# uw-math-ai/TheoremSearch

Hardware: AMD Instinct MI355X
Metric: queries/sec, brute-force top-10 over N x 768 theorem embeddings (higher is better)
Workload: dtype bf16; 1 GPU; 10000000x768 bf16 corpus, batch-256 queries, top-10 (BASELINE.json configs[2]); rows=10000000, dim=768, batch=256, k=10, searches_in_flight=1, parallelism=corpus row-sharded x1

## Files before the change

theoremsearch_amd/csrc/host.h:

```cpp
#pragma once
#include <hip/hip_runtime.h>

#include <algorithm>
#include <cmath>
#include <cctype>
#include <cstdarg>
#include <cstdio>
#include <cstdlib>
#include <cstring>
#include <atomic>
#include <memory>
#include <mutex>
#include <new>
#include <type_traits>
#include <vector>

#include "../../include/tsearch.h"
#include "common.h"
#include "scan_plan.h"
#include "anyd_plan.h"
#include "bias_plan.h"
#include "encoder_plan.h"
#include "meta_plan.h"
#include "dev_array.h"

using namespace ts;

inline thread_local char g_err[512] = "";

inline int fail(int code, const char* fmt, ...) {
    va_list ap;
    va_start(ap, fmt);
    vsnprintf(g_err, sizeof(g_err), fmt, ap);
    va_end(ap);
    return code;
}

#define HIP_TRY(expr)                                                                                   \
    do {                                                                                                \
        hipError_t e_ = (expr);                                                                         \
        if (e_ != hipSuccess)                                                                           \
            return fail(e_ == hipErrorOutOfMemory ? TS_ERR_NOMEM : TS_ERR_HIP, "%s failed: %s (%s:%d)", \
                        #expr, hipGetErrorString(e_), __FILE__, __LINE__);                              \
    } while (0)

#define DEV_TRY(expr) HIP_TRY((hipError_t)(expr))

#define TS_TRY(expr)            \
    do {                        \
        int rc_ = (expr);       \
        if (rc_ != TS_OK) return rc_; \
    } while (0)

template <auto Kernel, int Limit = 0, class... A>
inline int launch_lds(int dev, dim3 grid, dim3 block, int lds, hipStream_t st, const A&... args) {
    static std::atomic<int> raised[64];
    static std::mutex raise_mu;
    const int want = Limit ? Limit : lds;
    std::atomic<int>& have = raised[dev & 63];
    if (have.load(std::memory_order_acquire) < want) {
        std::lock_guard<std::mutex> lock(raise_mu);
        if (have.load(std::memory_order_relaxed) < want) {
            HIP_TRY(hipFuncSetAttribute((const void*)Kernel, hipFuncAttributeMaxDynamicSharedMemorySize, want));
            have.store(want, std::memory_order_release);
        }
    }
    Kernel<<<grid, block, lds, st>>>(args...);
    HIP_TRY(hipGetLastError());
    return TS_OK;
}

template <int V> using variant_c = std::integral_constant<int, V>;
template <int... Vs, class Go>
inline bool launch_variant(int variant, int* rc, Go&& go) {
    return ((variant == Vs && ((*rc = go(variant_c<Vs>{})), true)) || ...);
}

template <int... Vs, class Go>
inline int dispatch_value(int v, Go&& go) {
    int rc = TS_ERR_INVALID;
    if (!launch_variant<Vs...>(v, &rc, go)) return fail(rc, "internal: no kernel for the value %d", v);
    return rc;
}

enum Knob {
    K_MFMA_MIN_RANK, K_MFMA_VARIANT, K_MFMA_GROUPS, K_MFMA_GRID, K_MFMA_STAT, K_MFMA_STAT_CANDS, K_MFMA_TAIL_FIT,
    K_MFMA_NO_IDLE, K_MFMA_AHEAD, K_MFMA_TARGET_CANDS, K_MFMA_FIRST_ROWS, K_MFMA_TARGET_SPARSE, K_MFMA_RUN,
    K_MFMA_MIN_ROWS, K_MFMA_SHAPE, K_MFMA_F32, K_SCAN_GENERIC, K_SCAN_MAX_QUERIES, K_MFMA_BALANCE, K_PROBE_SPREAD, K_MFMA_SAMPLE,
    K_MFMA_PAIR, K_MFMA_PAIR_LAG, K_MFMA_SCREEN, K_MFMA_SCREEN_WIDE, K_MFMA_SCREEN_F32, K_MFMA_SCREEN_LATE, K_COUNT
};
inline const char* const kKnobNames[K_COUNT] = {
    "TS_MFMA_MIN_RANK", "TS_MFMA_VARIANT", "TS_MFMA_GROUPS", "TS_MFMA_GRID", "TS_MFMA_STAT", "TS_MFMA_STAT_CANDS",
    "TS_MFMA_TAIL_FIT", "TS_MFMA_NO_IDLE", "TS_MFMA_AHEAD", "TS_MFMA_TARGET_CANDS", "TS_MFMA_FIRST_ROWS",
    "TS_MFMA_TARGET_SPARSE", "TS_MFMA_RUN", "TS_MFMA_MIN_ROWS", "TS_MFMA_SHAPE", "TS_MFMA_F32", "TS_SCAN_GENERIC",
    "TS_SCAN_MAX_QUERIES", "TS_MFMA_BALANCE", "TS_PROBE_SPREAD", "TS_MFMA_SAMPLE", "TS_MFMA_PAIR", "TS_MFMA_PAIR_LAG",
    "TS_MFMA_SCREEN", "TS_MFMA_SCREEN_WIDE", "TS_MFMA_SCREEN_F32", "TS_MFMA_SCREEN_LATE"};
struct Knobs {
    int v[K_COUNT];
    bool set[K_COUNT];
    Knobs() {
        for (int i = 0; i < K_COUNT; ++i) {
            const char* e = getenv(kKnobNames[i]);
            set[i] = e && *e;
            v[i] = set[i] ? atoi(e) : 0;
        }
#ifndef TS_DIAG
        for (int i = 0; i < K_COUNT; ++i)
            if (diag_only((Knob)i)) { set[i] = false; v[i] = 0; }
#endif
    }
    static bool diag_only(Knob k) {
        return k == K_MFMA_VARIANT || k == K_MFMA_MIN_RANK || k == K_MFMA_GROUPS || k == K_MFMA_STAT_CANDS || k == K_MFMA_NO_IDLE ||
               k == K_MFMA_TARGET_CANDS || k == K_MFMA_TARGET_SPARSE || k == K_MFMA_MIN_ROWS || k == K_SCAN_GENERIC ||
               k == K_SCAN_MAX_QUERIES || k == K_PROBE_SPREAD;
    }
    int get(Knob k, int dflt) const { return set[k] ? v[k] : dflt; }
};

constexpr int kCandCap = 8192;
constexpr size_t kStageBytes = (size_t)256 << 20;

struct HipMem {
    static int alloc(void** p, size_t bytes) { return (int)hipMalloc(p, bytes ? bytes : 1); }
    static void free(void* p) { (void)hipFree(p); }
    static int zero(void* p, size_t bytes) { return (int)hipMemset(p, 0, bytes); }
};
template <class T> using DevArray = DevArrayOf<T, HipMem>;
using DevBuf = DevArray<void>;

struct IndexQueue {
    hipStream_t stream = nullptr;
    hipEvent_t order_ev = nullptr;
    bool ordered = false;
    std::vector<hipEvent_t> ev_pool;
    IndexQueue() = default;
    IndexQueue(const IndexQueue&) = delete;
    IndexQueue& operator=(const IndexQueue&) = delete;
    ~IndexQueue() {
        for (hipEvent_t e : ev_pool) hipEventDestroy(e);
        if (order_ev) hipEventDestroy(order_ev);
        if (stream) hipStreamDestroy(stream);
    }
};

struct ts_index : IndexQueue {
    int device = 0;
    int64_t n = 0, n_pad = 0, ld = 0, row_offset = 0;
    int d = 0, dtype = 0, metric = 0;
    int cu_count = 256;
    DevArray<void> rows;
    std::mutex mu;
    DevArray<void> stage;
    DevArray<void> qstore;      DevArray<float> qf32;
    DevArray<u64> cand;         DevArray<u32> count;         DevArray<float> thr;
    DevArray<u64> priv;         DevArray<u32> pcount;        int priv_writers = 0;
    DevArray<float> sample;
    bool rebalance_pending = false, rebalance_in_rerun = false; int rebalance_grid = 0;
    DevArray<int> fb_list;      DevArray<int> fb_count;      DevArray<u32> stat;
    DevArray<u64> partial;
    DevArray<u64> partial2;
    DevArray<float> res_scores; DevArray<int64_t> res_idx;   size_t res_cap = 0;
    DevArray<u32> mask_dev;
    DevArray<float> bias_dev;
    DevArray<u32> bias_hist;
    const float* active_bias = nullptr; float active_bias_w = 0.f;
    bool active_bias_matrix = false;
    DevArray<int64_t> id_map;
    bool borrowed = false;
    bool attached = false;
    ts_index* parent = nullptr;
    std::atomic<int> nviews{0};
    DevArray<void> rank_buf;
    DevArray<void> rank_many_buf;
    const u32* active_mask = nullptr;
    int64_t active_allowed = 0;
    Knobs knobs;
    hipStream_t last_stream = nullptr;
    DevArray<int64_t> part;     DevArray<unsigned> wg_ticks;
    int part_g = 0;             int64_t part_ntiles = -1;
// ... 53 lines not shown

inline hipEvent_t prof_begin(ts_index* ix, hipStream_t st, int64_t rows) {
    if (!ix->profiling) return nullptr;
    if (ix->ev_used + 2 > ix->ev_pool.size()) {
        if (ix->ev_pool.size() >= 16384) return nullptr;
        hipEvent_t a = nullptr, b = nullptr;
        if (hipEventCreate(&a) != hipSuccess) return nullptr;
        if (hipEventCreate(&b) != hipSuccess) { hipEventDestroy(a); return nullptr; }
        ix->ev_pool.push_back(a);
        ix->ev_pool.push_back(b);
    }
    hipEvent_t start = ix->ev_pool[ix->ev_used], stop = ix->ev_pool[ix->ev_used + 1];
    ix->ev_used += 2;
    ix->prof_rows = rows;
    hipEventRecord(start, st);
    return stop;
}
inline void prof_end(hipEvent_t stop, hipStream_t st) {
    if (stop) hipEventRecord(stop, st);
}

struct StreamScope {
    ts_index* ix = nullptr;
    hipStream_t st = nullptr;
    ~StreamScope() {
        if (!ix || !ix->order_ev) return;
        hipStreamCaptureStatus cap = hipStreamCaptureStatusNone;
        if (hipStreamIsCapturing(st, &cap) != hipSuccess) (void)hipGetLastError();
        if (cap != hipStreamCaptureStatusNone) return;
        if (hipEventRecord(ix->order_ev, st) == hipSuccess) {
            ix->last_stream = st;
            ix->ordered = true;
        } else {
            (void)hipGetLastError();
        }
    }
};
inline int enter_stream(ts_index* ix, void* stream, hipStream_t* out, StreamScope* scope) {
    hipStream_t st = stream ? (hipStream_t)stream : ix->stream;
    if (!ix->order_ev) HIP_TRY(hipEventCreateWithFlags(&ix->order_ev, hipEventDisableTiming));
    if (ix->ordered && ix->last_stream != st) HIP_TRY(hipStreamWaitEvent(st, ix->order_ev, 0));
    scope->ix = ix;
    scope->st = st;
    *out = st;
    return TS_OK;
}

inline int check_device(int device) {
    int c = 0;
    ts_device_count(&c);
    if (c <= 0) return fail(TS_ERR_NODEVICE, "no HIP device visible (libtsearch has no CPU path)");
    if (device < 0 || device >= c) return fail(TS_ERR_INVALID, "device %d out of range [0, %d)", device, c);
    return TS_OK;
}

static inline bool mfma_dim(int d) { return d == 384 || d == 512 || d == 768 || d == 1024; }
static inline bool two_level_search(const ts_index* ix) {
    return ix->knobs.get(K_MFMA_STAT, 1) != 0 && ix->knobs.get(K_MFMA_SAMPLE, 1) != 0;
}
static inline bool anyd_index(const ts_index* ix) {
    if (ix->dtype == TS_F32 && ix->knobs.get(K_MFMA_F32, 16) == 0) return false;
    return ix->ld == ix->d && anyd_served(ix->dtype, ix->d, two_level_search(ix));
}
static inline bool bias_index(const ts_index* ix) {
    if (ix->dtype == TS_F32 && ix->knobs.get(K_MFMA_F32, 16) == 0) return false;
    return ix->ld == ix->d && ix->n >= 1 && bias_served(ix->dtype, ix->d, two_level_search(ix));
}
static inline bool mfma_index(const ts_index* ix) {
    if (anyd_index(ix)) return true;
    if (ix->dtype == TS_BF16) return mfma_dim(ix->d);
    if (ix->knobs.get(K_MFMA_F32, 16) == 0) return false;
    return ix->d == 768 || ix->d == 1024 || ((ix->d == 384 || ix->d == 512) && two_level_search(ix));
}

static inline bool use_shape16(const ts_index* ix) {
    if (!mfma_dim(ix->d)) return false;
    const bool narrow = ix->d == 384 || ix->d == 512;
    const bool two_level = two_level_search(ix);
    if (ix->dtype == TS_F32) return ix->d != 768 || ix->knobs.get(K_MFMA_F32, 16) != 32;
    if (narrow && !two_level) return false;
    return ix->dtype == TS_BF16 && mfma_dim(ix->d) && ix->knobs.get(K_MFMA_SHAPE, 16) != 32;
}

namespace ts { struct MfmaArgs; }
int prep_dispatch(int src_dtype, int dst_dtype, bool normalize, const void* src, int64_t src_ld, void* dst, float* f32copy,
                  int64_t ld, int d, int64_t nrows, int64_t rows_total, hipStream_t st);
int scan_search(ts_index* ix, int nq, int k, float* out_scores, int64_t* out_idx, const int* qlist, const int* qcount,
                hipStream_t st, const float* qbuf = nullptr, const unsigned short* qb16 = nullptr);
struct QueryFeed {
    ts_index* ix = nullptr;
    const char* queries = nullptr;
    size_t row_bytes = 0;
    int q_dtype = 0;
    bool on_device = false, f32copy = false;
    hipStream_t st = nullptr;
    const void* at(int q0) const { return queries + (size_t)q0 * row_bytes; }
};
int query_feed_open(QueryFeed* f, ts_index* ix, const void* queries, int q_dtype, int q_on_device, int nq, bool f32copy, hipStream_t st);
int query_feed_block(const QueryFeed& f, int q0, int nb);
int mfma_block_queries(const ts_index* ix, int nq);
int bias_histogram(ts_index* ix, hipStream_t st);
int mfma_search(ts_index* ix, int nq, int k, float* out_scores, int64_t* out_idx, hipStream_t st, ts_search_stats* stats,
                const void* qmat, bool in_place);
int launch_pass_mfma16(int dev, int d, int nb, bool full_pass, int variant, int grid, hipStream_t st, const ts::MfmaArgs& a);
int launch_pass_mfma16_f32(int dev, int d, int nb, bool full_pass, int grid, hipStream_t st, const ts::MfmaArgs& a);
bool screen_usable(const ts_index* ix);
int screen_prepare(ts_index* ix, const void* qmat, int nq_launch, bool quantize_queries, hipStream_t st);
int screen_full_pass(ts_index* ix, int nb, int nq, int grid, int variant, bool ksplit, hipStream_t st, const ts::MfmaArgs& a);
int screen_tile_pass(ts_index* ix, int nb, int grid, int variant, hipStream_t st, const ts::MfmaArgs& a);
int screen_prepare_wide(ts_index* ix, const void* qmat, int nq_launch, bool quantize_queries, hipStream_t st);
int screen_full_pass_wide(ts_index* ix, int nb, int nq, int grid, int variant, bool ksplit, hipStream_t st, const ts::MfmaArgs& a);
int screen_tile_pass_wide(ts_index* ix, int nb, int grid, int variant, hipStream_t st, const ts::MfmaArgs& a);
int launch_screen8_late(int dev, int grid, hipStream_t st, const ts::MfmaArgs& a);
int screen_prepare_f32(ts_index* ix, const void* qmat, int nq_launch, hipStream_t st);
int screen_full_pass_f32(ts_index* ix, int nb, int nq, int grid, int variant, hipStream_t st, const ts::MfmaArgs& a);
int launch_pass_mfma_anyd(const ts_index* ix, int grid, hipStream_t st, const ts::MfmaArgs& a);
int launch_pass_mfma_anyd_biased(const ts_index* ix, int grid, hipStream_t st, const ts::MfmaArgs& a);
int launch_pass_mfma32(int dev, int d, int groups, bool full_pass, int variant, int grid, hipStream_t st, const ts::MfmaArgs& a);
int launch_pass_mfma32_f32(int dev, bool full_pass, int variant, int grid, hipStream_t st, const ts::MfmaArgs& a);
```

theoremsearch_amd/csrc/kernels_level.h:

```cpp
#pragma once
#include "kernels_select.h"

namespace ts {

struct LevelArgs {
    const u64* priv;
    const u32* pcount;
    int nwriters;
    int priv_cap;
    const u64* cand;
    u32* count;
    int cap;
    int kk;
    float* thr;
    int final_level;
    float z_tail;
    float tail_p;
    float tail_z;
    int min_fill;
    float* out_scores;
    int64_t* out_idx;
    int k_user;
    int64_t row_offset;
    const int64_t* id_map;
// ... 49 lines not shown
    TS_DPP_F64_STEP(TS_DPP_BCAST15, 0xa)
    TS_DPP_F64_STEP(TS_DPP_BCAST31, 0xc)
#undef TS_DPP_F64_STEP
    const u64 b = (u64)__double_as_longlong(v);
    const u32 lo = (u32)__builtin_amdgcn_readlane((int)(u32)b, 63), hi = (u32)__builtin_amdgcn_readlane((int)(u32)(b >> 32), 63);
    return __longlong_as_double((long long)(((u64)hi << 32) | lo));
}

constexpr int kFinalFast = 128;

__device__ __forceinline__ bool level_final_one_wave(const LevelArgs& a, int q) {
    if (!(a.final_level && a.nwriters == 0 && a.k_user <= kFinalFast)) return false;
    const u32 raw0 = a.count[q];
    if (!(raw0 <= (u32)kFinalFast && raw0 <= (u32)a.cap)) return false;
    if (threadIdx.x >= 64) return true;
    const int lane = threadIdx.x;
    u64 v[2];
#pragma unroll
    for (int r = 0; r < 2; ++r) v[r] = ((u32)(64 * r + lane) < raw0) ? a.cand[(int64_t)q * a.cap + 64 * r + lane] : 0ull;
    if (lane == 0) {
        a.count[q] = 0;
        a.stat_q[q] = raw0;
    }
    if ((int)raw0 < a.min_fill) {
        if (lane == 0) a.fb_list[atomicAdd(a.fb_count, 1)] = q;
        return true;
    }
    wave_sort_desc<u64, 2>(v, lane);
#pragma unroll
    for (int r = 0; r < 2; ++r) {
        const int i = 64 * r + lane;
        if (i < a.k_user) {
            const u64 key = v[r];
            a.out_scores[(int64_t)q * a.k_user + i] = key ? key_score(key) : -INFINITY;
            a.out_idx[(int64_t)q * a.k_user + i] = !key ? -1 : a.id_map ? a.id_map[key_row(key)] : (int64_t)key_row(key) + a.row_offset;
        }
    }
    return true;
}

template <int KR>
__global__ void __launch_bounds__(kLevelThreads) level_select_kernel(LevelArgs a) {
    extern __shared__ __attribute__((aligned(16))) unsigned char smem[];
    const SelectLds lds = SelectLds::carve(smem, kLevelSortMax);
    const int q = blockIdx.x;
    if (level_final_one_wave(a, q)) return;
    u32& fill = lds.ctr[kSelFill];
    u32& produced = lds.ctr[kSelProduced];
    u32& base_shared = lds.ctr[kSelSharedBase];
    if (threadIdx.x == 0) {
        fill = 0;
        produced = 0;
        lds.ctr[kSelShort] = 0;
    }
    for (int i = threadIdx.x; i < kLevelBins; i += blockDim.x) lds.hist[i] = 0;
    __syncthreads();
    for (int w = threadIdx.x; w < a.nwriters; w += blockDim.x) {
        const u32 made = a.pcount[(int64_t)q * a.nwriters + w];
        if (made == 0) continue;
        const u32 n = min(made, (u32)a.priv_cap);
        const u64* src = a.priv + ((int64_t)q * a.nwriters + w) * a.priv_cap;
        const u32 at = atomicAdd(&fill, n);
        atomicAdd(&produced, n);
        u64 v[32];
#pragma unroll
        for (int e = 0; e < 32; ++e) v[e] = ((u32)e < n) ? src[e] : 0ull;
#pragma unroll
        for (int e = 0; e < 32; ++e)
            if ((u32)e < n && at + e < (u32)kLevelSortMax) lds.keys[at + e] = v[e];
    }
    const u32 raw = a.count[q];
    const u32 ns = min(raw, (u32)a.cap);
    __syncthreads();
    if (threadIdx.x == 0) {
        base_shared = fill;
        fill += ns;
        produced += raw;
    }
    __syncthreads();
    for (u32 i = threadIdx.x; i < ns; i += blockDim.x)
        if (base_shared + i < (u32)kLevelSortMax) lds.keys[base_shared + i] = a.cand[(int64_t)q * a.cap + i];
    __syncthreads();
    const u32 total = fill;
    const bool lost = raw > (u32)a.cap || total > (u32)kLevelSortMax;
    const int cnt = (int)min(total, (u32)kLevelSortMax);
    const int kk = a.kk;
    constexpr int kTailM = 32;
    const bool tail_fit = !a.final_level && a.tail_p > 0.0f;
    const int kl = tail_fit ? max(kk, kTailM) : kk;

    double mean = 0.0, sd = 0.0;
    u64* best = lds_select_top<KR>(lds, cnt, kl, !a.final_level && a.z_tail > 0.0f && cnt >= 256, mean, sd);

    if (threadIdx.x == 0) a.count[q] = 0;
    if (!a.final_level) {
        const float thr = level_threshold(a, best, cnt, kk, tail_fit, mean, sd);
        if (threadIdx.x == 0) a.thr[q] = thr;
        return;
    }
    if (threadIdx.x == 0) a.stat_q[q] = produced;
    if (lost || (int)total < a.min_fill) {
        if (threadIdx.x == 0) a.fb_list[atomicAdd(a.fb_count, 1)] = q;
        return;
    }
    for (int i = threadIdx.x; i < a.k_user; i += blockDim.x) {
        const u64 key = best[i];
        a.out_scores[(int64_t)q * a.k_user + i] = key ? key_score(key) : -INFINITY;
        a.out_idx[(int64_t)q * a.k_user + i] = !key ? -1 : a.id_map ? a.id_map[key_row(key)] : (int64_t)key_row(key) + a.row_offset;
    }
}

constexpr int kSelCap = 1024;

constexpr int kSelThreads = 256;
template <int THREADS>
__global__ void __launch_bounds__(THREADS) sample_select_fast_kernel(LevelArgs a, const float* scores, int row_stride, float z_sel) {
    constexpr int NW = THREADS / 64;
    constexpr int J4 = kLevelSortMax / (4 * THREADS);
    __shared__ double red[2 * NW];
    __shared__ u32 wcount[2][NW];
    __shared__ __attribute__((aligned(16))) u32 surv[kSelCap];
    __shared__ __attribute__((aligned(16))) u64 best[kSelCap];
    __shared__ u32 nsurv;
    const int q = blockIdx.x;
    const int lane = threadIdx.x & 63, wave = threadIdx.x >> 6;
    if (threadIdx.x == 0) {
        a.count[q] = 0;
        nsurv = 0;
    }
    const float4* src = (const float4*)(scores + (int64_t)q * row_stride);
    const int n4 = row_stride >> 2;
    float v[4 * J4];
#pragma unroll
    for (int j = 0; j < J4; ++j) {
        const int i = j * THREADS + threadIdx.x;
        const float4 t = (i < n4) ? src[i] : make_float4(-INFINITY, -INFINITY, -INFINITY, -INFINITY);
        v[4 * j] = t.x; v[4 * j + 1] = t.y; v[4 * j + 2] = t.z; v[4 * j + 3] = t.w;
    }
    double s1 = 0.0, s2 = 0.0;
    u32 nl = 0;
    u32 o[4 * J4];
#pragma unroll
    for (int e = 0; e < 4 * J4; ++e) {
        const bool live = v[e] == v[e] && v[e] > -INFINITY;
        const double d = live ? (double)v[e] : 0.0;
        s1 += d;
        s2 += d * d;
        nl += (u32)__popcll(__ballot(live));
        o[e] = live ? ord_f32(v[e]) : 0u;
    }
    s1 = wave_total_f64(s1);
    s2 = wave_total_f64(s2);
    if (lane == 0) { red[2 * wave] = s1; red[2 * wave + 1] = s2; wcount[0][wave] = nl; }
    __syncthreads();
    double t1 = 0.0, t2 = 0.0;
    int cnt = 0;
#pragma unroll
    for (int w = 0; w < NW; ++w) { t1 += red[2 * w]; t2 += red[2 * w + 1]; cnt += (int)wcount[0][w]; }
    const double mean = cnt > 0 ? t1 / cnt : 0.0;
    const double sd = cnt > 0 ? sqrt(fmax(t2 / cnt - mean * mean, 0.0)) : 0.0;
    const int kk = a.kk;
    constexpr int kTailM = 32;
    const bool tail_fit = a.tail_p > 0.0f;
    const int kl = min(tail_fit ? max(kk, kTailM) : kk, kMaxK);

    int flip = 1;
    auto count_ge = [&](u32 cut) __attribute__((always_inline)) -> u32 {
        u32 c = 0;
#pragma unroll
        for (int e = 0; e < 4 * J4; ++e) c += (u32)__popcll(__ballot(o[e] >= cut));
        if (lane == 0) wcount[flip][wave] = c;
        __syncthreads();
        u32 tot = 0;
#pragma unroll
        for (int w = 0; w < NW; ++w) tot += wcount[flip][w];
        flip ^= 1;
        return tot;
    };
    const u32 want = (u32)min(kl, cnt);
    u32 cut = 1u, c = 0;
    bool found = want == 0;
    if (!found && sd > 0.0) {
        float z = z_sel;
        for (int t = 0; t < 3 && !found; ++t) {
            cut = max(ord_f32((float)(mean + (double)z * sd)), 1u);
            c = count_ge(cut);
            if (c < want) z -= 0.75f;
            else if (c > (u32)kSelCap) z += 0.75f;
            else found = true;
        }
    }
    if (!found) {
// ... 64 lines not shown
```

theoremsearch_amd/csrc/launch_screen8.hip:

```cpp
#include "launch_screen8_impl.h"

bool screen_usable(const ts_index* ix) {
    bool served = false;
    if (ix->dtype == TS_BF16) served = ix->d == 768 || (ix->d == 1024 && ix->knobs.get(K_MFMA_SCREEN_WIDE, 0) != 0);
    else if (ix->dtype == TS_F32)
        served = (ix->d == 768 || ix->d == 1024) && ix->knobs.get(K_MFMA_SCREEN_F32, 0) != 0 && ix->knobs.get(K_MFMA_F32, 16) != 32 &&
                 two_level_search(ix);
    return served && ix->ld == ix->d && use_shape16(ix) && !ix->borrowed && !ix->attached && ix->knobs.get(K_MFMA_SCREEN, 1) != 0;
}

int screen_prepare(ts_index* ix, const void* qmat, int nq_launch, bool quantize_queries, hipStream_t st) {
    if (ix->dtype == TS_F32) return screen_prepare_f32(ix, qmat, nq_launch, st);
    if (ix->d == 1024) return screen_prepare_wide(ix, qmat, nq_launch, quantize_queries, st);
    return screen_prepare_w<768>(ix, qmat, nq_launch, quantize_queries, st);
}

int screen_full_pass(ts_index* ix, int nb, int nq, int grid, int variant, bool ksplit, hipStream_t st, const MfmaArgs& a) {
    if (ix->dtype == TS_F32) return screen_full_pass_f32(ix, nb, nq, grid, variant, st, a);
    if (ix->d == 1024) return screen_full_pass_wide(ix, nb, nq, grid, variant, ksplit, st, a);
    return screen_full_pass_w<768>(ix, nb, nq, grid, variant, ksplit, st, a);
}

int screen_tile_pass(ts_index* ix, int nb, int grid, int variant, hipStream_t st, const MfmaArgs& a) {
    if (ix->d == 1024) return screen_tile_pass_wide(ix, nb, grid, variant, st, a);
    return screen_tile_pass_w<768>(ix, nb, grid, variant, st, a);
}
```

theoremsearch_amd/csrc/launch_screen8_impl.h:

```cpp
#pragma once
#include "host.h"
#include "kernels_screen8.h"

template <int W, int NB>
static int launch_screen8(int dev, int grid, int variant, hipStream_t st, const MfmaArgs& a) {
    constexpr int D = W / 2;
    constexpr int lds = Mfma16Dims<D>::kLds + kMfma16StageBytes;
#ifdef TS_DIAG
    constexpr bool kDiag = NB == 4;
#else
    constexpr bool kDiag = false;
#endif
    static_assert(lds <= 160 * 1024, "DMA ring + staged candidates must fit the CU's LDS");
    const bool masked = a.row_mask != nullptr;
    auto go = [&](auto v) { return launch_lds<mfma16_topk_kernel<D, NB, decltype(v)::value, false>>(dev, grid, kMfmaThreads, lds, st, a); };
    int rc;
    if constexpr (kDiag)
        if (launch_variant<kVariantScreenNoEpilogue, kVariantScreenStamps, kVariantScreenClockProbe, kVariantScreenDmaOnly, kVariantScreenTestOnly>(variant, &rc, go)) return rc;
    return masked ? go(variant_c<kVariantScreenMasked>{}) : go(variant_c<kVariantScreen>{});
}

template <int W, class QuantizeTiles, class QuantizeQueries>
static int screen_prepare_with(ts_index* ix, bool quantize_queries, QuantizeTiles&& quantize_tiles, QuantizeQueries&& quantize_query_rows) {
    const int64_t tiles = ix->n_pad / kTileRows;
    if (ix->scr_pad != ix->n_pad) {
        ix->scr_pad = 0;
        DEV_TRY(remake(ix->scr_rows, (size_t)ix->n_pad * W, ix->scr_tile, (size_t)tiles * 16));
        ix->scr_pad = ix->n_pad;
        ix->scr_lo = 0;
        ix->scr_hi = ix->n_pad;
    }
    if (ix->scr_lo < ix->scr_hi) {
        const int64_t t0 = ix->scr_lo / kTileRows;
        const int64_t t1 = std::min(tiles, (ix->scr_hi + kTileRows - 1) / kTileRows);
        for (int64_t t = t0; t < t1; t += 1 << 20) {
            quantize_tiles(t, (unsigned)std::min<int64_t>(1 << 20, t1 - t));
            HIP_TRY(hipGetLastError());
        }
        ix->scr_lo = ix->scr_hi = 0;
    }
    DEV_TRY(ix->scr_q.need((size_t)kMfmaQ * W));
    DEV_TRY(ix->scr_qmeta.need((size_t)kMfmaQ * 16));
    DEV_TRY(ix->scr_cand.need((size_t)kMfmaQ * kScreenCap * 8));
    DEV_TRY(ix->scr_count.need((size_t)kMfmaQ * 4));
    if (quantize_queries) {
        quantize_query_rows();
        HIP_TRY(hipGetLastError());
    }
    return TS_OK;
}

template <int W>
static int screen_prepare_w(ts_index* ix, const void* qmat, int nq_launch, bool quantize_queries, hipStream_t st) {
    return screen_prepare_with<W>(
        ix, quantize_queries,
        [&](int64_t tile0, unsigned nblk) {
            quantize_tiles_kernel<W><<<nblk, 256, 0, st>>>(ix->rows.as<const unsigned short>(), ix->scr_rows.as<signed char>(), ix->scr_tile.as<float4>(), tile0);
        },
        [&] {
            quantize_queries_kernel<W><<<kMfmaQ, 64, 0, st>>>((const unsigned short*)qmat, std::min(nq_launch, kMfmaQ), ix->scr_q.as<signed char>(),
                                                           ix->scr_qmeta.as<float4>(), ix->scr_count);
        });
}

template <int W>
static int screen_tile_pass_w(ts_index* ix, int nb, int grid, int variant, hipStream_t st, const MfmaArgs& a, bool late = false) {
    MfmaArgs s = a;
    s.corpus = ix->scr_rows.as<const unsigned short>();
    s.q = ix->scr_q.as<const unsigned short>();
    s.cand = ix->scr_cand;
    s.count = ix->scr_count;
    s.cap = kScreenCap;
    s.scr_tile = ix->scr_tile.as<const float4>();
    s.scr_q = ix->scr_qmeta.as<const float4>();
    if constexpr (W == 768)
        if (late && nb == 4 && variant == kVariantProduct && s.row_mask == nullptr) return launch_screen8_late(ix->device, grid, st, s);
    switch (nb) {
        case 1: return launch_screen8<W, 1>(ix->device, grid, variant, st, s);
        case 2: return launch_screen8<W, 2>(ix->device, grid, variant, st, s);
        case 3: return launch_screen8<W, 3>(ix->device, grid, variant, st, s);
        case 4: return launch_screen8<W, 4>(ix->device, grid, variant, st, s);
        default: return fail(TS_ERR_INTERNAL, "no int8 screen with %d query blocks per wave", nb);
    }
}

template <int W>
static int screen_full_pass_w(ts_index* ix, int nb, int nq, int grid, int variant, bool ksplit, hipStream_t st, const MfmaArgs& a) {
    TS_TRY(screen_tile_pass_w<W>(ix, nb, grid, variant, st, a, W == 768 && ix->dtype == TS_BF16 && ix->knobs.get(K_MFMA_SCREEN_LATE, 1) != 0));
    ScreenRescoreArgs r;
    r.rows = ix->rows.as<const unsigned short>();
    r.q = a.q;
    r.thr = a.thr;
    r.scand = ix->scr_cand;
    r.scount = ix->scr_count;
    r.cand = a.cand;
    r.count = a.count;
    r.cap = a.cap;
    if constexpr (W == 1024) {
        if (ksplit) screen_rescore_kernel<W, true><<<dim3((unsigned)nq, kRescoreY), 256, 0, st>>>(r);
        else screen_rescore_kernel<W, false><<<dim3((unsigned)nq, kRescoreY), 256, 0, st>>>(r);
    } else {
        if (ksplit) return fail(TS_ERR_INTERNAL, "the k-split rescore is a form of the d = 1024 pass, not of d = %d", W);
        screen_rescore_kernel<W, false><<<dim3((unsigned)nq, kRescoreY), 256, 0, st>>>(r);
    }
    HIP_TRY(hipGetLastError());
    return TS_OK;
}
```

theoremsearch_amd/csrc/search_mfma.hip:

```cpp
#include "host.h"
#include "kernels_mfma.h"
#include "kernels_mfma16.h"
#include "mfma16_variants.h"
#include "kernels_mfma_f32.h"
#include "kernels_sample.h"
#include "kernels_sample_biased.h"
#include "kernels_level.h"

struct Level { int64_t stride, ntiles; int run; };

static double normal_tail_z(double p) {
    if (p <= 0.0) return 8.0;
    if (p >= 0.5) return 0.0;
    const double q = std::sqrt(-2.0 * std::log(p));
    static const double c[] = {-7.784894002430293e-03, -3.223964580411365e-01, -2.400758277161838e+00,
                               -2.549732539343734e+00, 4.374664141464968e+00, 2.938163982698783e+00};
    static const double d[] = {7.784695709041462e-03, 3.224671290700398e-01, 2.445134137142996e+00, 3.754408661907416e+00};
    if (p < 0.02425)
        return -(((((c[0] * q + c[1]) * q + c[2]) * q + c[3]) * q + c[4]) * q + c[5]) /
               ((((d[0] * q + d[1]) * q + d[2]) * q + d[3]) * q + 1.0);
    static const double a[] = {-3.969683028665376e+01, 2.209460984245205e+02, -2.759285104469687e+02,
                               1.383577518672690e+02, -3.066479806614716e+01, 2.506628277459239e+00};
    static const double b[] = {-5.447609879822406e+01, 1.615858368580409e+02, -1.556989798598866e+02,
                               6.680131188771972e+01, -1.328068155288572e+01};
// ... 289 lines not shown
            ix->probe_units = (double)h[2];
            if (ix->knobs.get(K_PROBE_SPREAD, 0)) {
                std::vector<double> us;
                double xm[8] = {0}, xn[8] = {0};
                for (int w = 0; w < grid; ++w)
                    if (h[w * 4 + 1] > 0) {
                        us.push_back((double)h[w * 4 + 1] * 0.01);
                        xm[w & 7] += us.back();
                        xn[w & 7] += 1;
                    }
                std::sort(us.begin(), us.end());
                fprintf(stderr, "[tsearch probe] tile loop per workgroup: min %.1f us, median %.1f, max %.1f; mean by id %% 8:", us.front(),
                        us[us.size() / 2], us.back());
                for (int x = 0; x < 8; ++x) fprintf(stderr, " %.1f", xm[x] / std::max(1.0, xn[x]));
                fprintf(stderr, "\n");
            }
        }
    } else if (p.shape16 && (variant == kVariantStamps || (p.screen && variant == kVariantScreenStamps))) {
        std::vector<unsigned long long> h((size_t)grid * 16);
        HIP_TRY(hipStreamSynchronize(st));
        HIP_TRY(hipMemcpy(h.data(), dbg, h.size() * 8, hipMemcpyDeviceToHost));
        const double units = (double)(p.lv.back().ntiles * (variant == kVariantScreenStamps ? (ix->d == 1024 ? Mfma16Dims<512>::kUnits : Mfma16Dims<384>::kUnits) : MfmaDims<768>::kUnits)) / grid;
        for (int wv = 0; wv < 4; ++wv) {
            double tot = 0, vm = 0, bar = 0, dma = 0;
            for (int w = wv; w < grid * 4; w += 4) { tot += h[w * 4]; vm += h[w * 4 + 1]; bar += h[w * 4 + 2]; dma += h[w * 4 + 3]; }
            if (variant == kVariantScreenStamps)
                fprintf(stderr, "[tsearch stamps8] wave %d per tile: total %.0f cycles, vmcnt wait %.0f, barrier wait %.0f, tile tail %.0f (drain to end of epilogue; stamp cost ~40 each included)\n",
                        wv, tot / grid / units, vm / grid / units, bar / grid / units, dma / grid / units);
            else
                fprintf(stderr, "[tsearch stamps16] wave %d per unit: total %.0f cycles, vmcnt wait %.0f, barrier wait %.0f, DMA issue %.0f (6 pieces; stamp cost ~40 each included)\n",
                        wv, tot / grid / units, vm / grid / units, bar / grid / units, dma / grid / units);
        }
    } else if (!p.shape16) {
        std::vector<unsigned long long> h((size_t)grid * 16);
        HIP_TRY(hipStreamSynchronize(st));
        HIP_TRY(hipMemcpy(h.data(), dbg, h.size() * 8, hipMemcpyDeviceToHost));
        for (int wv = 0; wv < 4; ++wv) {
            double tot = 0, vm = 0, bar = 0, units = 0;
            for (int w = wv; w < grid * 4; w += 4) { tot += h[w * 4]; vm += h[w * 4 + 1]; bar += h[w * 4 + 2]; units += h[w * 4 + 3]; }
            fprintf(stderr, "[tsearch stamps] wave %d per unit: total %.0f cycles, vmcnt wait %.0f, barrier wait %.0f (units/wave %.0f)\n",
                    wv, tot / units, vm / units, bar / units, units / grid);
        }
    }
    return TS_OK;
}
#endif

static int mfma_level(ts_index* ix, const MfmaPlan& p, size_t i, int nq, int k, float* out_scores, int64_t* out_idx, const void* qmat,
                      hipStream_t st) {
    const Level& lv = p.lv[i];
    const bool full_pass = (i + 1 == p.lv.size());
    MfmaArgs a;
    a.corpus = ix->rows.as<const unsigned short>();
    a.n = ix->n;
    a.ntiles = lv.ntiles;
    a.tile_stride = lv.stride;
    a.run = lv.run;
    a.q = (const unsigned short*)qmat;
    a.thr = ix->thr;
    a.nq = ix->knobs.get(K_MFMA_NO_IDLE, 0) ? 256 : nq;
    a.row_mask = ix->active_mask;
    a.ahead = ix->knobs.get(K_MFMA_AHEAD, 0);
    a.priv = ix->priv;
    a.pcount = ix->pcount;
    a.cand = ix->cand;
    a.count = ix->count;
    a.cap = kCandCap;
    a.first_level = (i == 0) ? 1 : 0;
    a.nq_real = nq;
    a.fb_count = ix->fb_count;
    a.part = (p.balance && full_pass) ? ix->part : nullptr;
    a.wg_ticks = (p.balance && full_pass) ? ix->wg_ticks : nullptr;
    a.pair = (p.pair && full_pass) ? (p.ksplit_form ? 2 : 1) : 0;
    const bool paced = a.pair && p.pair_lag > 0;
    a.pair_pos = paced ? ix->pair_pos : nullptr;
    a.pair_lag = paced ? p.pair_lag : 0;
    a.dbg = nullptr;
    a.scr_tile = nullptr;
    a.scr_q = nullptr;
#ifdef TS_DIAG
    if (variant_gets_dbg(p.variant) && !p.anyd) a.dbg = ix->dbg;
#endif
    if (p.anyd && !full_pass) return fail(TS_ERR_INTERNAL, "the general-width matrix kernel has no sparse level");
    hipEvent_t stop = full_pass ? prof_begin(ix, st, ix->n) : nullptr;
    int rc;
    if (p.biased) rc = launch_pass_mfma_anyd_biased(ix, p.grid, st, a);
    else if (p.anyd) rc = launch_pass_mfma_anyd(ix, p.grid, st, a);
    else if (p.screen && full_pass) rc = screen_full_pass(ix, p.nb16, nq, p.grid, p.screen_diag ? p.variant : kVariantProduct, p.ksplit_form, st, a);
    else if (ix->dtype == TS_F32 && p.shape16) rc = launch_pass_mfma16_f32(ix->device, ix->d, p.nb16, full_pass, p.grid, st, a);
    else if (ix->dtype == TS_F32) rc = launch_pass_mfma32_f32(ix->device, full_pass, p.variant, p.grid, st, a);
    else if (p.shape16) rc = launch_pass_mfma16(ix->device, ix->d, p.nb16, full_pass, p.variant, p.grid, st, a);
    else rc = launch_pass_mfma32(ix->device, ix->d, p.groups, full_pass, p.variant, p.grid, st, a);
    prof_end(stop, st);
    TS_TRY(rc);
#ifdef TS_DIAG
    if (a.dbg && full_pass) TS_TRY(mfma_diag_readout(ix, p, a.dbg, st));
#endif
    LevelArgs l;
    memset(&l, 0, sizeof(l));
    l.priv = ix->priv;
    l.pcount = ix->pcount;
    l.nwriters = ((p.shape16 || p.anyd) && full_pass) ? 0 : p.nwriters;
    l.priv_cap = p.priv_cap;
    l.cand = ix->cand;
    l.count = ix->count;
    l.cap = kCandCap;
    l.kk = p.kk;
    l.thr = ix->thr;
    l.final_level = full_pass;
    l.z_tail = full_pass ? 0.0f : p.z_tail;
    l.tail_p = full_pass ? 0.0f : p.tail_p;
    l.tail_z = (float)normal_tail_z(std::min(0.25, 32.0 / p.sample_rows));
    l.min_fill = (int)std::min<int64_t>(k, p.pop);
    l.out_scores = out_scores;
    l.out_idx = out_idx;
    l.k_user = k;
    l.row_offset = ix->row_offset;
    l.id_map = ix->id_map;
    l.fb_list = ix->fb_list;
    l.fb_count = ix->fb_count;
    l.stat_q = ix->stat;
    l.nq = nq;
    if (p.kk <= 64) return launch_lds<level_select_kernel<1>>(ix->device, nq, kLevelThreads, kLevelLds, st, l);
    return launch_lds<level_select_kernel<4>>(ix->device, nq, kLevelThreads, kLevelLds, st, l);
}

int mfma_search(ts_index* ix, int nq, int k, float* out_scores, int64_t* out_idx, hipStream_t st, ts_search_stats* stats,
                       const void* qmat, bool in_place) {
    const MfmaPlan p = mfma_plan(ix, nq, k);
    TS_TRY(mfma_scratch(ix, p, st));
    if (p.screen) TS_TRY(screen_prepare(ix, qmat, p.nq_launch, !(p.dense0 && p.screen_rider), st));
    for (size_t i = 0; i < p.lv.size(); ++i) {
        if (i == 0 && p.dense0) TS_TRY(mfma_sample(ix, p, nq, qmat, st));
        else TS_TRY(mfma_level(ix, p, i, nq, k, out_scores, out_idx, qmat, st));
    }
    ix->rebalance_pending = p.balance;
    ix->rebalance_grid = p.wgs;
    ix->rebalance_in_rerun = !(p.dense_sample && p.lv.size() == 2);
    if (!in_place) TS_TRY(scan_search(ix, nq, k, out_scores, out_idx, ix->fb_list, ix->fb_count, st));
    else if (ix->dtype == TS_F32) TS_TRY(scan_search(ix, nq, k, out_scores, out_idx, ix->fb_list, ix->fb_count, st, (const float*)qmat));
    else TS_TRY(scan_search(ix, nq, k, out_scores, out_idx, ix->fb_list, ix->fb_count, st, nullptr, (const unsigned short*)qmat));
    if (stats) {
        stats->levels = (int)p.lv.size();
        stats->screened = p.screen ? 1 : 0;
    }
    return TS_OK;
}
```

Before: 156,200 queries/s.

## Fuse screened rescore and final top-k select into one finish kernel

For the bf16 d=768 screened search, the rescore of screened candidates and the final level select now run in a single kernel per query instead of two launches. Candidates are rescored with MFMA into LDS keys and selected in place, with a wave-sort fast path for small candidate counts, so the intermediate candidate list no longer round-trips through global memory and one launch is removed. The fused kernel uses 1024 threads and a large LDS footprint, which may lower occupancy compared with the separate rescore kernel.

```diff
diff --git a/theoremsearch_amd/csrc/host.h b/theoremsearch_amd/csrc/host.h
--- a/theoremsearch_amd/csrc/host.h
+++ b/theoremsearch_amd/csrc/host.h
@@ -87,14 +87,15 @@
     K_MFMA_MIN_RANK, K_MFMA_VARIANT, K_MFMA_GROUPS, K_MFMA_GRID, K_MFMA_STAT, K_MFMA_STAT_CANDS, K_MFMA_TAIL_FIT,
     K_MFMA_NO_IDLE, K_MFMA_AHEAD, K_MFMA_TARGET_CANDS, K_MFMA_FIRST_ROWS, K_MFMA_TARGET_SPARSE, K_MFMA_RUN,
     K_MFMA_MIN_ROWS, K_MFMA_SHAPE, K_MFMA_F32, K_SCAN_GENERIC, K_SCAN_MAX_QUERIES, K_MFMA_BALANCE, K_PROBE_SPREAD, K_MFMA_SAMPLE,
-    K_MFMA_PAIR, K_MFMA_PAIR_LAG, K_MFMA_SCREEN, K_MFMA_SCREEN_WIDE, K_MFMA_SCREEN_F32, K_MFMA_SCREEN_LATE, K_COUNT
+    K_MFMA_PAIR, K_MFMA_PAIR_LAG, K_MFMA_SCREEN, K_MFMA_SCREEN_WIDE, K_MFMA_SCREEN_F32, K_MFMA_SCREEN_LATE,
+    K_MFMA_FINISH, K_COUNT
 };
 inline const char* const kKnobNames[K_COUNT] = {
     "TS_MFMA_MIN_RANK", "TS_MFMA_VARIANT", "TS_MFMA_GROUPS", "TS_MFMA_GRID", "TS_MFMA_STAT", "TS_MFMA_STAT_CANDS",
     "TS_MFMA_TAIL_FIT", "TS_MFMA_NO_IDLE", "TS_MFMA_AHEAD", "TS_MFMA_TARGET_CANDS", "TS_MFMA_FIRST_ROWS",
     "TS_MFMA_TARGET_SPARSE", "TS_MFMA_RUN", "TS_MFMA_MIN_ROWS", "TS_MFMA_SHAPE", "TS_MFMA_F32", "TS_SCAN_GENERIC",
     "TS_SCAN_MAX_QUERIES", "TS_MFMA_BALANCE", "TS_PROBE_SPREAD", "TS_MFMA_SAMPLE", "TS_MFMA_PAIR", "TS_MFMA_PAIR_LAG",
-    "TS_MFMA_SCREEN", "TS_MFMA_SCREEN_WIDE", "TS_MFMA_SCREEN_F32", "TS_MFMA_SCREEN_LATE"};
+    "TS_MFMA_SCREEN", "TS_MFMA_SCREEN_WIDE", "TS_MFMA_SCREEN_F32", "TS_MFMA_SCREEN_LATE", "TS_MFMA_FINISH"};
 struct Knobs {
     int v[K_COUNT];
     bool set[K_COUNT];
@@ -314,7 +315,7 @@
     return ix->dtype == TS_BF16 && mfma_dim(ix->d) && ix->knobs.get(K_MFMA_SHAPE, 16) != 32;
 }
 
-namespace ts { struct MfmaArgs; }
+namespace ts { struct MfmaArgs; struct LevelArgs; struct ScreenRescoreArgs; }
 int prep_dispatch(int src_dtype, int dst_dtype, bool normalize, const void* src, int64_t src_ld, void* dst, float* f32copy,
                   int64_t ld, int d, int64_t nrows, int64_t rows_total, hipStream_t st);
 int scan_search(ts_index* ix, int nq, int k, float* out_scores, int64_t* out_idx, const int* qlist, const int* qcount,
@@ -338,7 +339,10 @@
 int launch_pass_mfma16_f32(int dev, int d, int nb, bool full_pass, int grid, hipStream_t st, const ts::MfmaArgs& a);
 bool screen_usable(const ts_index* ix);
 int screen_prepare(ts_index* ix, const void* qmat, int nq_launch, bool quantize_queries, hipStream_t st);
-int screen_full_pass(ts_index* ix, int nb, int nq, int grid, int variant, bool ksplit, hipStream_t st, const ts::MfmaArgs& a);
+int screen_full_pass(ts_index* ix, int nb, int nq, int grid, int variant, bool ksplit, hipStream_t st, const ts::MfmaArgs& a,
+                     const ts::LevelArgs* finish = nullptr);
+bool screen_finish_served(const ts_index* ix);
+int launch_screen_finish(int dev, int nq, hipStream_t st, const ts::ScreenRescoreArgs& r, const ts::LevelArgs& l);
 int screen_tile_pass(ts_index* ix, int nb, int grid, int variant, hipStream_t st, const ts::MfmaArgs& a);
 int screen_prepare_wide(ts_index* ix, const void* qmat, int nq_launch, bool quantize_queries, hipStream_t st);
 int screen_full_pass_wide(ts_index* ix, int nb, int nq, int grid, int variant, bool ksplit, hipStream_t st, const ts::MfmaArgs& a);
diff --git a/theoremsearch_amd/csrc/kernels_level.h b/theoremsearch_amd/csrc/kernels_level.h
--- a/theoremsearch_amd/csrc/kernels_level.h
+++ b/theoremsearch_amd/csrc/kernels_level.h
@@ -155,32 +155,7 @@
         if (base_shared + i < (u32)kLevelSortMax) lds.keys[base_shared + i] = a.cand[(int64_t)q * a.cap + i];
     __syncthreads();
     const u32 total = fill;
-    const bool lost = raw > (u32)a.cap || total > (u32)kLevelSortMax;
-    const int cnt = (int)min(total, (u32)kLevelSortMax);
-    const int kk = a.kk;
-    constexpr int kTailM = 32;
-    const bool tail_fit = !a.final_level && a.tail_p > 0.0f;
-    const int kl = tail_fit ? max(kk, kTailM) : kk;
-
-    double mean = 0.0, sd = 0.0;
-    u64* best = lds_select_top<KR>(lds, cnt, kl, !a.final_level && a.z_tail > 0.0f && cnt >= 256, mean, sd);
-
-    if (threadIdx.x == 0) a.count[q] = 0;
-    if (!a.final_level) {
-        const float thr = level_threshold(a, best, cnt, kk, tail_fit, mean, sd);
-        if (threadIdx.x == 0) a.thr[q] = thr;
-        return;
-    }
-    if (threadIdx.x == 0) a.stat_q[q] = produced;
-    if (lost || (int)total < a.min_fill) {
-        if (threadIdx.x == 0) a.fb_list[atomicAdd(a.fb_count, 1)] = q;
-        return;
-    }
-    for (int i = threadIdx.x; i < a.k_user; i += blockDim.x) {
-        const u64 key = best[i];
-        a.out_scores[(int64_t)q * a.k_user + i] = key ? key_score(key) : -INFINITY;
-        a.out_idx[(int64_t)q * a.k_user + i] = !key ? -1 : a.id_map ? a.id_map[key_row(key)] : (int64_t)key_row(key) + a.row_offset;
-    }
+#include "kernels_level_tail.inc"
 }
 
 constexpr int kSelCap = 1024;
diff --git a/theoremsearch_amd/csrc/kernels_level_tail.inc b/theoremsearch_amd/csrc/kernels_level_tail.inc
--- /dev/null
+++ b/theoremsearch_amd/csrc/kernels_level_tail.inc
@@ -0,0 +1,26 @@
+    const bool lost = raw > (u32)a.cap || total > (u32)kLevelSortMax;
+    const int cnt = (int)min(total, (u32)kLevelSortMax);
+    const int kk = a.kk;
+    constexpr int kTailM = 32;
+    const bool tail_fit = !a.final_level && a.tail_p > 0.0f;
+    const int kl = tail_fit ? max(kk, kTailM) : kk;
+
+    double mean = 0.0, sd = 0.0;
+    u64* best = lds_select_top<KR>(lds, cnt, kl, !a.final_level && a.z_tail > 0.0f && cnt >= 256, mean, sd);
+
+    if (threadIdx.x == 0) a.count[q] = 0;
+    if (!a.final_level) {
+        const float thr = level_threshold(a, best, cnt, kk, tail_fit, mean, sd);
+        if (threadIdx.x == 0) a.thr[q] = thr;
+        return;
+    }
+    if (threadIdx.x == 0) a.stat_q[q] = produced;
+    if (lost || (int)total < a.min_fill) {
+        if (threadIdx.x == 0) a.fb_list[atomicAdd(a.fb_count, 1)] = q;
+        return;
+    }
+    for (int i = threadIdx.x; i < a.k_user; i += blockDim.x) {
+        const u64 key = best[i];
+        a.out_scores[(int64_t)q * a.k_user + i] = key ? key_score(key) : -INFINITY;
+        a.out_idx[(int64_t)q * a.k_user + i] = !key ? -1 : a.id_map ? a.id_map[key_row(key)] : (int64_t)key_row(key) + a.row_offset;
+    }
diff --git a/theoremsearch_amd/csrc/kernels_screen8_finish.h b/theoremsearch_amd/csrc/kernels_screen8_finish.h
--- /dev/null
+++ b/theoremsearch_amd/csrc/kernels_screen8_finish.h
@@ -0,0 +1,128 @@
+#pragma once
+#include "kernels_level.h"
+#include "kernels_screen8.h"
+
+namespace ts {
+
+constexpr int kFinishThreads = 1024;
+constexpr int kFinishWaves = kFinishThreads / 64;
+constexpr int kFinishSelectBytes = kLevelSortMax * 8 + kLevelSmall * 8 + kFinishWaves * kMaxK * 8 + kLevelBins * 4 + kSelCtrWords * 4;
+template <int W> constexpr int kFinishLds = kFinishSelectBytes + W * 2;
+static_assert(kFinishSelectBytes % 16 == 0, "the query's fragments are read 16 bytes at a time");
+static_assert(kFinishLds<768> <= 160 * 1024, "select areas + query must fit the CU's LDS");
+
+template <int W, int KR>
+__global__ void __launch_bounds__(kFinishThreads) screen_finish_kernel(ScreenRescoreArgs r, LevelArgs a) {
+    static_assert(W == 768, "the default screened search: 24 row fragments per lane beside the chain fit 128 VGPRs");
+    constexpr int kSteps = W / 32;
+    extern __shared__ __attribute__((aligned(16))) unsigned char smem[];
+    SelectLds lds;
+    lds.keys = (u64*)smem;
+    lds.small = lds.keys + kLevelSortMax;
+    lds.wlists = lds.small + kLevelSmall;
+    lds.hist = (u32*)(lds.wlists + kFinishWaves * kMaxK);
+    lds.ctr = lds.hist + kLevelBins;
+    const bf16x8* qs = (const bf16x8*)(smem + kFinishSelectBytes);
+    const int q = blockIdx.x;
+    const int lane = threadIdx.x & 63, wave = threadIdx.x >> 6;
+    const int r16 = lane & 15, kq = lane >> 4;
+    u32& produced = lds.ctr[kSelProduced];
+    uint4 qpiece = make_uint4(0u, 0u, 0u, 0u);
+    if (threadIdx.x < W / 8) qpiece = ((const uint4*)(r.q + (int64_t)q * W))[threadIdx.x];
+    const u32 sraw = r.scount[q];
+    if (sraw > (u32)kScreenCap) {
+        if (threadIdx.x == 0) {
+            a.count[q] = 0;
+            a.stat_q[q] = (u32)a.cap + 1u;
+            a.fb_list[atomicAdd(a.fb_count, 1)] = q;
+        }
+        return;
+    }
+    const int m = (int)sraw;
+    const int nchunks = (m + 15) >> 4;
+    auto entry = [&](int cc) { const int e = 16 * cc + r16; return e < m ? (u32)r.scand[(int64_t)q * kScreenCap + e] : 0u; };
+    int c = wave;
+    u32 row = 0;
+    frag16 rf[kSteps];
+    if (c < nchunks) {
+        row = entry(c);
+        const frag16* pr = (const frag16*)(r.rows + (int64_t)row * W + 8 * kq);
+#pragma unroll
+        for (int ks = 0; ks < kSteps; ++ks) rf[ks] = pr[4 * ks];
+    }
+    const float thr = r.thr[q];
+    if (threadIdx.x == 0) {
+        lds.ctr[kSelFill] = 0;
+        produced = 0;
+        lds.ctr[kSelShort] = 0;
+    }
+    for (int i = threadIdx.x; i < kLevelBins; i += kFinishThreads) lds.hist[i] = 0;
+    if (threadIdx.x < W / 8) ((uint4*)(smem + kFinishSelectBytes))[threadIdx.x] = qpiece;
+    __syncthreads();
+    const u32 room = (u32)min(a.cap, kLevelSortMax);
+    while (c < nchunks) {
+        const int cn = c + kFinishWaves;
+        const u32 row_next = cn < nchunks ? entry(cn) : 0u;
+        f32x4 acc;
+        bf16x8 qf[kSteps];
+        int issued = 0;
+#pragma unroll
+        for (int ks = 0; ks < kSteps; ++ks) {
+            const int upto = min(kSteps, ks + 1 + min(ks + 1, 3));
+#pragma unroll
+            for (int f = 0; f < kSteps; ++f)
+                if (f >= issued && f < upto) qf[f] = qs[4 * f + kq];
+            issued = upto;
+            if (ks == 0) mfma16_v_first(acc, rf[0], qf[0]);
+            else mfma16_v(acc, rf[ks], qf[ks]);
+        }
+        asm volatile("s_nop 15\n\ts_nop 3" : "+v"(acc));
+        u32 rr[4];
+#pragma unroll
+        for (int i = 0; i < 4; ++i) rr[i] = (u32)__shfl((int)row, 4 * kq + i);
+        if (r16 == (q & 15)) {
+#pragma unroll
+            for (int i = 0; i < 4; ++i) {
+                const float s = acc[i];
+                if (16 * c + 4 * kq + i < m && s >= thr) {
+                    const u32 pos = atomicAdd(&produced, 1u);
+                    if (pos < room) lds.keys[pos] = make_key(s, rr[i]);
+                }
+            }
+        }
+        c = cn;
+        row = row_next;
+        if (c < nchunks) {
+            const frag16* pr = (const frag16*)(r.rows + (int64_t)row * W + 8 * kq);
+#pragma unroll
+            for (int ks = 0; ks < kSteps; ++ks) rf[ks] = pr[4 * ks];
+        }
+    }
+    __syncthreads();
+    const u32 raw = produced;
+    const u32 total = min(raw, (u32)a.cap);
+    if (a.k_user <= kFinalFast && raw <= (u32)kFinalFast && raw <= (u32)a.cap) {
+        if (threadIdx.x >= 64) return;
+        u64 v[2];
+#pragma unroll
+        for (int j = 0; j < 2; ++j) v[j] = ((u32)(64 * j + lane) < raw) ? lds.keys[64 * j + lane] : 0ull;
+        if (lane == 0) {
+            a.count[q] = 0;
+            a.stat_q[q] = raw;
+        }
+        if ((int)raw < a.min_fill) {
+            if (lane == 0) a.fb_list[atomicAdd(a.fb_count, 1)] = q;
+            return;
+        }
+        wave_sort_desc<u64, 2>(v, lane);
+#pragma unroll
+        for (int j = 0; j < 2; ++j) {
+            const int i = 64 * j + lane;
+            if (i < a.k_user) write_result_slot(a.out_scores, a.out_idx, a.k_user, a.id_map, a.row_offset, q, i, v[j]);
+        }
+        return;
+    }
+#include "kernels_level_tail.inc"
+}
+
+}
diff --git a/theoremsearch_amd/csrc/launch_screen8.hip b/theoremsearch_amd/csrc/launch_screen8.hip
--- a/theoremsearch_amd/csrc/launch_screen8.hip
+++ b/theoremsearch_amd/csrc/launch_screen8.hip
@@ -15,10 +15,14 @@
     return screen_prepare_w<768>(ix, qmat, nq_launch, quantize_queries, st);
 }
 
-int screen_full_pass(ts_index* ix, int nb, int nq, int grid, int variant, bool ksplit, hipStream_t st, const MfmaArgs& a) {
+bool screen_finish_served(const ts_index* ix) { return ix->dtype == TS_BF16 && ix->d == 768 && ix->knobs.get(K_MFMA_FINISH, 1) != 0; }
+
+int screen_full_pass(ts_index* ix, int nb, int nq, int grid, int variant, bool ksplit, hipStream_t st, const MfmaArgs& a,
+                     const LevelArgs* finish) {
+    if (finish && (!screen_finish_served(ix) || ksplit)) return fail(TS_ERR_INTERNAL, "no one-launch finish for this screened search");
     if (ix->dtype == TS_F32) return screen_full_pass_f32(ix, nb, nq, grid, variant, st, a);
     if (ix->d == 1024) return screen_full_pass_wide(ix, nb, nq, grid, variant, ksplit, st, a);
-    return screen_full_pass_w<768>(ix, nb, nq, grid, variant, ksplit, st, a);
+    return screen_full_pass_w<768>(ix, nb, nq, grid, variant, ksplit, st, a, finish);
 }
 
 int screen_tile_pass(ts_index* ix, int nb, int grid, int variant, hipStream_t st, const MfmaArgs& a) {
diff --git a/theoremsearch_amd/csrc/launch_screen8_finish.hip b/theoremsearch_amd/csrc/launch_screen8_finish.hip
--- /dev/null
+++ b/theoremsearch_amd/csrc/launch_screen8_finish.hip
@@ -0,0 +1,8 @@
+#include "host.h"
+#include "kernels_screen8_finish.h"
+
+int launch_screen_finish(int dev, int nq, hipStream_t st, const ScreenRescoreArgs& r, const LevelArgs& l) {
+    if (!l.final_level || l.nwriters != 0) return fail(TS_ERR_INTERNAL, "the screen's finish is the final select of the shared lists only");
+    if (l.kk <= 64) return launch_lds<screen_finish_kernel<768, 1>>(dev, nq, kFinishThreads, kFinishLds<768>, st, r, l);
+    return launch_lds<screen_finish_kernel<768, 4>>(dev, nq, kFinishThreads, kFinishLds<768>, st, r, l);
+}
diff --git a/theoremsearch_amd/csrc/launch_screen8_impl.h b/theoremsearch_amd/csrc/launch_screen8_impl.h
--- a/theoremsearch_amd/csrc/launch_screen8_impl.h
+++ b/theoremsearch_amd/csrc/launch_screen8_impl.h
@@ -85,7 +85,8 @@
 }
 
 template <int W>
-static int screen_full_pass_w(ts_index* ix, int nb, int nq, int grid, int variant, bool ksplit, hipStream_t st, const MfmaArgs& a) {
+static int screen_full_pass_w(ts_index* ix, int nb, int nq, int grid, int variant, bool ksplit, hipStream_t st, const MfmaArgs& a,
+                              const LevelArgs* finish = nullptr) {
     TS_TRY(screen_tile_pass_w<W>(ix, nb, grid, variant, st, a, W == 768 && ix->dtype == TS_BF16 && ix->knobs.get(K_MFMA_SCREEN_LATE, 1) != 0));
     ScreenRescoreArgs r;
     r.rows = ix->rows.as<const unsigned short>();
@@ -101,6 +102,7 @@
         else screen_rescore_kernel<W, false><<<dim3((unsigned)nq, kRescoreY), 256, 0, st>>>(r);
     } else {
         if (ksplit) return fail(TS_ERR_INTERNAL, "the k-split rescore is a form of the d = 1024 pass, not of d = %d", W);
+        if (finish) return launch_screen_finish(ix->device, nq, st, r, *finish);
         screen_rescore_kernel<W, false><<<dim3((unsigned)nq, kRescoreY), 256, 0, st>>>(r);
     }
     HIP_TRY(hipGetLastError());
diff --git a/theoremsearch_amd/csrc/search_mfma.hip b/theoremsearch_amd/csrc/search_mfma.hip
--- a/theoremsearch_amd/csrc/search_mfma.hip
+++ b/theoremsearch_amd/csrc/search_mfma.hip
@@ -395,20 +395,6 @@
     if (variant_gets_dbg(p.variant) && !p.anyd) a.dbg = ix->dbg;
 #endif
     if (p.anyd && !full_pass) return fail(TS_ERR_INTERNAL, "the general-width matrix kernel has no sparse level");
-    hipEvent_t stop = full_pass ? prof_begin(ix, st, ix->n) : nullptr;
-    int rc;
-    if (p.biased) rc = launch_pass_mfma_anyd_biased(ix, p.grid, st, a);
-    else if (p.anyd) rc = launch_pass_mfma_anyd(ix, p.grid, st, a);
-    else if (p.screen && full_pass) rc = screen_full_pass(ix, p.nb16, nq, p.grid, p.screen_diag ? p.variant : kVariantProduct, p.ksplit_form, st, a);
-    else if (ix->dtype == TS_F32 && p.shape16) rc = launch_pass_mfma16_f32(ix->device, ix->d, p.nb16, full_pass, p.grid, st, a);
-    else if (ix->dtype == TS_F32) rc = launch_pass_mfma32_f32(ix->device, full_pass, p.variant, p.grid, st, a);
-    else if (p.shape16) rc = launch_pass_mfma16(ix->device, ix->d, p.nb16, full_pass, p.variant, p.grid, st, a);
-    else rc = launch_pass_mfma32(ix->device, ix->d, p.groups, full_pass, p.variant, p.grid, st, a);
-    prof_end(stop, st);
-    TS_TRY(rc);
-#ifdef TS_DIAG
-    if (a.dbg && full_pass) TS_TRY(mfma_diag_readout(ix, p, a.dbg, st));
-#endif
     LevelArgs l;
     memset(&l, 0, sizeof(l));
     l.priv = ix->priv;
@@ -434,6 +420,22 @@
     l.fb_count = ix->fb_count;
     l.stat_q = ix->stat;
     l.nq = nq;
+    const bool finish = p.screen && full_pass && !p.screen_diag && !p.ksplit_form && l.nwriters == 0 && screen_finish_served(ix);
+    hipEvent_t stop = full_pass ? prof_begin(ix, st, ix->n) : nullptr;
+    int rc;
+    if (p.biased) rc = launch_pass_mfma_anyd_biased(ix, p.grid, st, a);
+    else if (p.anyd) rc = launch_pass_mfma_anyd(ix, p.grid, st, a);
+    else if (p.screen && full_pass) rc = screen_full_pass(ix, p.nb16, nq, p.grid, p.screen_diag ? p.variant : kVariantProduct, p.ksplit_form, st, a, finish ? &l : nullptr);
+    else if (ix->dtype == TS_F32 && p.shape16) rc = launch_pass_mfma16_f32(ix->device, ix->d, p.nb16, full_pass, p.grid, st, a);
+    else if (ix->dtype == TS_F32) rc = launch_pass_mfma32_f32(ix->device, full_pass, p.variant, p.grid, st, a);
+    else if (p.shape16) rc = launch_pass_mfma16(ix->device, ix->d, p.nb16, full_pass, p.variant, p.grid, st, a);
+    else rc = launch_pass_mfma32(ix->device, ix->d, p.groups, full_pass, p.variant, p.grid, st, a);
+    prof_end(stop, st);
+    TS_TRY(rc);
+#ifdef TS_DIAG
+    if (a.dbg && full_pass) TS_TRY(mfma_diag_readout(ix, p, a.dbg, st));
+#endif
+    if (finish) return TS_OK;
     if (p.kk <= 64) return launch_lds<level_select_kernel<1>>(ix->device, nq, kLevelThreads, kLevelLds, st, l);
     return launch_lds<level_select_kernel<4>>(ix->device, nq, kLevelThreads, kLevelLds, st, l);
 }
```

Result: no change. 156,800 queries/s, median of 2 (+0.4%).
